# tl32rodan/DCVC

Hardware: AMD Instinct MI355X
Metric: encode+decode fps @1920x1080 per GPU; bpp bit-exact + PSNR Δ<1e-4 dB vs ref (higher is better)
Workload: dtype f32 (convs on split-fp16 f16x3 MFMA, fp32 accumulation); 1 GPU; C3 DCVC-DC RGB 1920x1080 (pad 1920x1088) IP=32 write mode; gop=32, precision=split, q_index=0, stream_part=8, parallelism=sequence-sharded x1, 3 GOP lane(s) per GPU, lanes=3, step=one frame on each of 3 lane(s)

## Files before the change

dcvc_amd/csrc/hip/slffn.hip:

```cpp
#include "common.h"
#include "split.h"

#include <cstring>

namespace {

constexpr int kNW = 4, kNT = kNW * 64;

constexpr int HS = 64;
#ifndef SLFFN_PB384
#define SLFFN_PB384 2
#endif
#ifndef SLDC_PB384
#define SLDC_PB384 2
#endif
constexpr int kOob = 0x7fffffe0;

struct LP {
  const float *x;
  int npix, xcs, xco, xbytes;
  float *y;
  int ycs, yco, ybytes;
  const uint16_t *w1, *w2;
  int w1bytes, w2bytes;
// ... 372 lines not shown
  return (c == 192 || c == 384) && hidden > 0 && hidden % HS == 0;
}

extern "C" int64_t dcvc_internal_lffn_pack(const float *w1, const float *w2, int c, int hidden, void *out) {
  if (!dcvc_internal_lffn_supported(c, hidden)) return DCVC_HIP_EINVAL;
  const int64_t n1 = (int64_t)hidden * c * 2, n2 = (int64_t)c * hidden * 2;
  if (!out) return n1 + n2;
  uint16_t *o = reinterpret_cast<uint16_t *>(out);
  pack_frags(w1, hidden, c, o);
  pack_frags(w2, c, hidden, o + n1);
  return n1 + n2;
}

extern "C" int dcvc_internal_lffn(const dcvc_ffn_args *a, void *stream) {
  if (!dcvc_internal_lffn_supported(a->c, a->hidden)) return DCVC_HIP_EUNSUPPORTED;
  const int64_t npix = (int64_t)a->x.H * a->x.W;
  if (npix <= 0) return DCVC_HIP_OK;
  auto bytes = [&](int cs, int co) { return (npix * cs - co) * 4; };
  if (bytes(a->x.cstride, a->x.coff) > 0x7fff0000 || bytes(a->y.cstride, a->y.coff) > 0x7fff0000)
    return DCVC_HIP_EUNSUPPORTED;
  LP p{};
  p.ovf = dcvc_internal_split_flag();
  p.x = reinterpret_cast<const float *>(a->x.ptr);
  p.npix = (int)npix;
  p.xcs = a->x.cstride;
  p.xco = a->x.coff;
  p.xbytes = (int)bytes(a->x.cstride, a->x.coff);
  p.y = reinterpret_cast<float *>(a->y.ptr);
  p.ycs = a->y.cstride;
  p.yco = a->y.coff;
  p.ybytes = (int)bytes(a->y.cstride, a->y.coff);
  const int64_t n1 = (int64_t)a->hidden * a->c * 2;
  p.w1 = reinterpret_cast<const uint16_t *>(a->w);
  p.w2 = p.w1 + n1;
  p.w1bytes = (int)(n1 * 2);
  p.w2bytes = (int)(n1 * 2);
  p.b1 = a->b1;
  p.b2 = a->b2;
  p.scale = a->scale;
  p.hidden = a->hidden;
  p.slope = a->slope;
  hipStream_t st = reinterpret_cast<hipStream_t>(stream);
  return a->c == 384 ? run<384, SLFFN_PB384>(p, st) : run<192, 2>(p, st);
}

extern "C" int64_t dcvc_frag_pack_weights(const float *w, int rows, int k, void *out) {
  if (!w || rows <= 0 || k <= 0 || rows % 16 || k % 32) return DCVC_HIP_EINVAL;
  if (out && !host_split_range_ok(w, (int64_t)rows * k)) return DCVC_HIP_EINVAL;
  const int64_t n = (int64_t)rows * k * 2;
  if (out) pack_frags(w, rows, k, reinterpret_cast<uint16_t *>(out));
  return n;
}

extern "C" int dcvc_dw_conv2_split(const dcvc_dwc_args *a, void *stream) {
  if (!a || !a->t.ptr || !a->r.ptr || !a->y.ptr || !a->w9 || !a->bdw || !a->w2 || !a->b2) return DCVC_HIP_EINVAL;
  const int c = a->c;
  if (a->t.dtype != DCVC_F32 || a->r.dtype != DCVC_F32 || a->y.dtype != DCVC_F32 || a->t.C != c || a->r.C != c ||
      a->y.C != c || a->t.H != a->y.H || a->t.W != a->y.W || a->r.H != a->y.H || a->r.W != a->y.W)
    return DCVC_HIP_EINVAL;
  if (c != 192 && c != 384 && c != 128) return DCVC_HIP_EUNSUPPORTED;
  auto al = [](const dcvc_tensor &v) { return (uintptr_t)v.ptr % 16 == 0 && v.cstride % 4 == 0 && v.coff % 4 == 0; };
  if (!al(a->t) || !al(a->r) || !al(a->y) || a->t.cstride % 8 || a->t.coff % 8) return DCVC_HIP_EUNSUPPORTED;
  const int64_t npix = (int64_t)a->t.H * a->t.W;
  if (npix <= 0) return DCVC_HIP_OK;
  auto bytes = [&](const dcvc_tensor &v) { return (npix * v.cstride - v.coff) * 4; };
  if (bytes(a->t) > 0x7fff0000 || bytes(a->r) > 0x7fff0000 || bytes(a->y) > 0x7fff0000) return DCVC_HIP_EUNSUPPORTED;
  DP p{};
  p.ovf = dcvc_internal_split_flag();
  p.t = reinterpret_cast<const float *>(a->t.ptr);
  p.npix = (int)npix;
  p.H = a->t.H;
  p.W = a->t.W;
  p.tcs = a->t.cstride;
  p.tco = a->t.coff;
  p.tbytes = (int)bytes(a->t);
  p.r = reinterpret_cast<const float *>(a->r.ptr);
  p.rcs = a->r.cstride;
  p.rco = a->r.coff;
  p.rbytes = (int)bytes(a->r);
  p.y = reinterpret_cast<float *>(a->y.ptr);
  p.ycs = a->y.cstride;
  p.yco = a->y.coff;
  p.ybytes = (int)bytes(a->y);
  p.w9 = a->w9;
  p.bdw = a->bdw;
  p.w2 = reinterpret_cast<const uint16_t *>(a->w2);
  p.w2bytes = (int)((int64_t)c * c * 2 * 2);
  p.b2 = a->b2;
  hipStream_t st = reinterpret_cast<hipStream_t>(stream);
  return c == 384 ? run_dc<384, SLDC_PB384>(p, st) : c == 192 ? run_dc<192, 2>(p, st) : run_dc<128, 2>(p, st);
}
```

dcvc_amd/hip.py:

```python
import ctypes
import os
import threading

import numpy as np
import torch

from ._native import NativeError, hip_lib, check

F32, BF16 = 0, 1
F16X3 = 2
ACT_NONE, ACT_LRELU, ACT_CLAMP01, ACT_ROUND = 0, 1, 2, 3
IN_NONE, IN_LRELU, IN_GATE = 0, 1, 2

_TORCH = {F32: torch.float32, BF16: torch.bfloat16}
_CNAME = {F32: "f32", BF16: "bf16", F16X3: "f16x3"}
_CODE = {torch.float32: F32, torch.bfloat16: BF16}


class CTensor(ctypes.Structure):
    _fields_ = [("ptr", ctypes.c_void_p), ("dtype", ctypes.c_int), ("H", ctypes.c_int),
                ("W", ctypes.c_int), ("C", ctypes.c_int), ("cstride", ctypes.c_int),
                ("coff", ctypes.c_int)]


class CDcbArgs(ctypes.Structure):
    _fields_ = [("x", CTensor), ("y", CTensor), ("cin", ctypes.c_int), ("cout", ctypes.c_int),
                ("gated", ctypes.c_int),
                ("w_conv1", ctypes.c_void_p), ("ld_conv1", ctypes.c_int), ("b_conv1", ctypes.c_void_p),
                ("w_dw", ctypes.c_void_p), ("b_dw", ctypes.c_void_p),
                ("w_conv2", ctypes.c_void_p), ("ld_conv2", ctypes.c_int), ("b_conv2", ctypes.c_void_p),
                ("w_adaptor", ctypes.c_void_p), ("ld_adaptor", ctypes.c_int), ("b_adaptor", ctypes.c_void_p),
                ("w_ffn1", ctypes.c_void_p), ("ld_ffn1", ctypes.c_int), ("b_ffn1", ctypes.c_void_p),
                ("w_ffn2", ctypes.c_void_p), ("ld_ffn2", ctypes.c_int), ("b_ffn2", ctypes.c_void_p),
                ("scale", ctypes.c_void_p), ("slope_dc", ctypes.c_float), ("slope_ffn", ctypes.c_float)]


class CConvArgs(ctypes.Structure):
    _fields_ = [("x", CTensor), ("y", CTensor), ("w", ctypes.c_void_p), ("bias", ctypes.c_void_p),
                ("cin", ctypes.c_int), ("cout", ctypes.c_int), ("kh", ctypes.c_int), ("kw", ctypes.c_int),
                ("stride", ctypes.c_int), ("pad", ctypes.c_int), ("compute", ctypes.c_int),
                ("in_op", ctypes.c_int), ("in_slope", ctypes.c_float), ("act", ctypes.c_int),
                ("slope", ctypes.c_float), ("shuffle", ctypes.c_int), ("scale", ctypes.c_void_p),
                ("res", CTensor), ("res2", CTensor)]


class CFfnArgs(ctypes.Structure):
    _fields_ = [("x", CTensor), ("y", CTensor), ("c", ctypes.c_int), ("hidden", ctypes.c_int),
                ("w", ctypes.c_void_p), ("b1", ctypes.c_void_p), ("b2", ctypes.c_void_p),
                ("scale", ctypes.c_void_p), ("slope", ctypes.c_float)]


class CDcArgs(ctypes.Structure):
    _fields_ = [("x", CTensor), ("y", CTensor), ("cin", ctypes.c_int), ("cout", ctypes.c_int),
                ("adaptor", ctypes.c_int), ("w", ctypes.c_void_p), ("b1", ctypes.c_void_p), ("wdw", ctypes.c_void_p),
                ("bdw", ctypes.c_void_p), ("b2", ctypes.c_void_p), ("ba", ctypes.c_void_p), ("slope", ctypes.c_float)]


class CDwcArgs(ctypes.Structure):
    _fields_ = [("t", CTensor), ("r", CTensor), ("y", CTensor), ("c", ctypes.c_int), ("w9", ctypes.c_void_p),
                ("bdw", ctypes.c_void_p), ("w2", ctypes.c_void_p), ("b2", ctypes.c_void_p)]


_T = CTensor
_vp, _i, _f = ctypes.c_void_p, ctypes.c_int, ctypes.c_float
HIP_SYMBOLS = [
    ("dcvc_conv_pack_weights", ctypes.c_int64, [_vp, _i, _i, _i, _i, _i, _vp]),
    ("dcvc_conv2d", _i, [ctypes.POINTER(CConvArgs), _vp]),
    ("dcvc_set_option", _i, [ctypes.c_char_p, _i]),
    ("dcvc_get_option", _i, [ctypes.c_char_p, ctypes.POINTER(_i)]),
    ("dcvc_split_range_flag", _i, [_vp]),
    ("dcvc_last_kernel", ctypes.c_char_p, []),
    ("dcvc_depthconv_block", _i, [ctypes.POINTER(CDcbArgs), _vp]),
    ("dcvc_ffn_pack_weights", ctypes.c_int64, [_vp, _vp, _i, _i, _vp]),
    ("dcvc_conv_ffn", _i, [ctypes.POINTER(CFfnArgs), _vp]),
    ("dcvc_dc_pack_weights", ctypes.c_int64, [_vp, _vp, _vp, _i, _i, _vp]),
    ("dcvc_depth_conv_split", _i, [ctypes.POINTER(CDcArgs), _vp]),
    ("dcvc_frag_pack_weights", ctypes.c_int64, [_vp, _i, _i, _vp]),
    ("dcvc_dw_conv2_split", _i, [ctypes.POINTER(CDwcArgs), _vp]),
    ("dcvc_dwconv3x3", _i, [_T, _T, _vp, _vp, _vp]),
    ("dcvc_flow_warp", _i, [_T, _T, _T, _vp, _vp, _vp]),
    ("dcvc_offset_diversity", _i, [_T, _T, _T, _T, _vp, _vp, _vp, _vp, _f, _vp]),
    ("dcvc_offset_diversity_workspace", ctypes.c_int64, [_i, _i]),
    ("dcvc_offset_diversity_ws", _i, [_T, _T, _T, _T, _vp, _vp, _vp, _vp, _f, _vp, ctypes.c_int64, _vp]),
    ("dcvc_resize2x", _i, [_T, _T, _i, _f, _vp]),
    ("dcvc_pool2x2", _i, [_T, _T, _i, _vp]),
    ("dcvc_add", _i, [_T, _T, _T, _vp]),
    ("dcvc_copy", _i, [_T, _T, _vp]),
    ("dcvc_pad_replicate", _i, [_T, _T, _vp]),
    ("dcvc_frame_to_nhwc", _i, [_vp, _i, _i, _T, _vp]),
    ("dcvc_frame_to_nhwc_zero_pad", _i, [_vp, _i, _i, _T, _vp]),
    ("dcvc_yuv420_to_nhwc", _i, [_vp, _vp, _i, _i, _T, _vp]),
    ("dcvc_frame_sse_workspace", ctypes.c_int64, []),
    ("dcvc_frame_sse", _i, [_T, _vp, _vp, _i, _i, _i, _vp, _vp, _vp]),
    ("dcvc_recon_to_u8", _i, [_T, _i, _i, _i, _vp, _vp]),
    ("dcvc_yuv420_to_rgb_nhwc", _i, [_vp, _vp, _i, _i, _T, _vp, _vp]),
    ("dcvc_rgb_to_yuv420_planes", _i, [_vp, _i, _i, _vp, _vp, _vp]),
    ("dcvc_yuv420f_to_nhwc", _i, [_vp, _vp, _i, _i, _T, _vp]),
    ("dcvc_frame_sse_f32", _i, [_T, _vp, _vp, _i, _i, _i, _vp, _vp, _vp]),
    ("dcvc_recon_to_u8_cross", _i, [_T, _i, _i, _i, _vp, _vp]),
    ("dcvc_quadtree_encode_step", _i, [_T, _T, _T, _i, _T, _T, _vp, _vp, _f, _f, _vp]),
    ("dcvc_quadtree_indexes_step", _i, [_T, _T, _i, _vp, _f, _f, _vp]),
    ("dcvc_quadtree_decode_step", _i, [_T, _T, _i, _vp, _T, _T, _vp]),
    ("dcvc_nhwc_to_symbols", _i, [_T, _vp, _vp]),
    ("dcvc_symbols_to_nhwc", _i, [_vp, _T, _vp]),
    ("dcvc_quadtree_estimate_step", _i, [_T, _T, _T, _i, _T, _T, _vp, _i, _vp]),
    ("dcvc_factorized_bits", _i, [_T, _vp, _vp, _vp]),
    ("dcvc_sum_f32", _i, [_vp, ctypes.c_int64, _vp, _vp]),
    ("dcvc_dual_prior_encode_step", _i, [_T, _T, _T, _i, _T, _vp, _vp, _vp, _f, _f, _vp]),
    ("dcvc_dual_prior_indexes_step", _i, [_T, _T, _i, _vp, _f, _f, _vp]),
    ("dcvc_dual_prior_decode_step", _i, [_T, _T, _i, _vp, _T, _vp, _vp]),
    ("dcvc_dual_prior_estimate_step", _i, [_T, _T, _T, _i, _T, _vp, _vp, _i, _f, _vp]),
    ("dcvc_channel_div", _i, [_T, _vp, _T, _vp]),
    ("dcvc_fill", _i, [_T, _f, _vp]),
# ... 318 lines not shown
        w1 = w1.detach().float().cpu().reshape(w1.shape[0], -1).contiguous().numpy()
        w2 = w2.detach().float().cpu().reshape(w2.shape[0], -1).contiguous().numpy()
        self.hidden, self.c = w1.shape
        dev = _device(device)
        self.w = _pack(lib().dcvc_ffn_pack_weights, w1, w2, self.c, self.hidden, device=dev)
        self.b1 = b1.detach().float().contiguous().to(dev)
        self.b2 = b2.detach().float().contiguous().to(dev)


class DcW:

    def __init__(self, w1, b1, w9c, bdw, w2, b2, wa=None, ba=None, device=None):
        f = lambda w: w.detach().float().cpu().reshape(w.shape[0], -1).contiguous().numpy()
        w1n, w2n = f(w1), f(w2)
        wan = f(wa) if wa is not None else None
        self.cin, self.cout = w1n.shape[0], w2n.shape[0]
        dev = _device(device)
        self.w = _pack(lib().dcvc_dc_pack_weights, w1n, w2n, wan, self.cin, self.cout, device=dev)
        g = lambda t: t.detach().float().contiguous().to(dev)
        self.b1, self.w9c, self.bdw, self.b2 = g(b1), g(w9c), g(bdw), g(b2)
        self.ba = g(ba) if wa is not None else None


class DwcW:

    def __init__(self, w9c, bdw, w2, b2, device=None):
        w = w2.detach().float().cpu().reshape(w2.shape[0], -1).contiguous().numpy()
        self.c = int(w.shape[0])
        dev = _device(device)
        self.w2 = _pack(lib().dcvc_frag_pack_weights, w, self.c, self.c, device=dev)
        g = lambda t: t.detach().float().contiguous().to(dev)
        self.w9c, self.bdw, self.b2 = g(w9c), g(bdw), g(b2)


def dw_conv2_split(dwc, t, r, y=None):
    if y is None:
        y = empty(t.H, t.W, dwc.c, F32, t.buf.device)
    a = CDwcArgs()
    a.t, a.r, a.y, a.c = t.c(), r.c(), y.c(), dwc.c
    a.w9, a.bdw, a.w2, a.b2 = dwc.w9c.data_ptr(), dwc.bdw.data_ptr(), dwc.w2.data_ptr(), dwc.b2.data_ptr()
    e0 = _t0()
    rc = lib().dcvc_dw_conv2_split(ctypes.byref(a), stream())
    if rc == UNSUPPORTED:
        return None
    check(rc, "dw_conv2_split")
    if e0 is not None:
        n = t.H * t.W
        kname = lib().dcvc_last_kernel().decode()
        _t1(e0, kname.split("<")[0], 2 * n * dwc.c * (9 + dwc.c), n * dwc.c * 4 * 3 + dwc.w2.numel() * 2,
            f"{kname} | dw+conv2 {dwc.c} {t.H}x{t.W} f16x3")
    return y


def depth_conv_split(dw, x, y=None, slope=0.01):
    if y is None:
        y = empty(x.H, x.W, dw.cout, F32, x.buf.device)
    a = CDcArgs()
    a.x, a.y = x.c(), y.c()
    a.cin, a.cout, a.adaptor = dw.cin, dw.cout, 1 if dw.ba is not None else 0
    a.w, a.b1, a.wdw, a.bdw, a.b2 = dw.w.data_ptr(), dw.b1.data_ptr(), dw.w9c.data_ptr(), dw.bdw.data_ptr(), \
        dw.b2.data_ptr()
    a.ba = dw.ba.data_ptr() if dw.ba is not None else None
    a.slope = slope
    e0 = _t0()
    r = lib().dcvc_depth_conv_split(ctypes.byref(a), stream())
    if r == UNSUPPORTED:
        return None
    check(r, "depth_conv_split")
    if e0 is not None:
        n = x.H * x.W
        kname = lib().dcvc_last_kernel().decode()
        fl = 2 * n * (dw.cin * dw.cin + 9 * dw.cin + dw.cin * dw.cout * (2 if dw.ba is not None else 1))
        _t1(e0, kname.split("<")[0], fl, n * (dw.cin + dw.cout) * 4 + dw.w.numel() * 2,
            f"{kname} | depthconv {dw.cin}->{dw.cout} {x.H}x{x.W} f16x3")
    return y


def conv_ffn(fw, x, y=None, scale=None, slope=0.1):
    if y is None:
        y = empty(x.H, x.W, x.C, F32, x.buf.device)
    a = CFfnArgs()
    a.x, a.y = x.c(), y.c()
    a.c, a.hidden = fw.c, fw.hidden
    a.w, a.b1, a.b2 = fw.w.data_ptr(), fw.b1.data_ptr(), fw.b2.data_ptr()
    a.scale = scale.data_ptr() if scale is not None else None
    a.slope = slope
    e0 = _t0()
    r = lib().dcvc_conv_ffn(ctypes.byref(a), stream())
    if r == UNSUPPORTED:
        return None
    check(r, "conv_ffn")
    if e0 is not None:
        n = x.H * x.W
        kname = lib().dcvc_last_kernel().decode()
        _t1(e0, kname.split("<")[0], 4 * n * fw.c * fw.hidden, n * fw.c * 4 * 3 + fw.w.numel() * 2,
            f"{kname} | ffn {fw.c}->{fw.hidden}->{fw.c} {x.H}x{x.W} f16x3")
    return y


def depthconv_block(blk, x, y, scale=None):
    a = CDcbArgs()
    a.x, a.y = x.c(), y.c()
    a.cin, a.cout, a.gated = blk.conv1.cin, blk.ffn2.cout, 1 if blk.gated else 0
    cp = lambda cw: (cw.w.data_ptr(), cw.w.numel() // cw.cout, cw.b.data_ptr())
    a.w_conv1, a.ld_conv1, a.b_conv1 = cp(blk.conv1)
    a.w_dw, a.b_dw = blk.dw[0].data_ptr(), blk.dw[1].data_ptr()
# ... 340 lines not shown
```

dcvc_amd/layers.py:

```python
import torch

from . import hip as K
from .hip import Act, F32, BF16, F16X3, ACT_LRELU, ACT_NONE, IN_LRELU, IN_GATE


FUSE_DCB = True
FUSE_FFN = True
FUSE_DC = True
DW128 = True
SDC_SHAPES = {(64, 48, True), (48, 32, True), (32, 64, True), (64, 64, False), (48, 48, False), (32, 32, False)}


class Precision:
    def __init__(self, feat, feat_compute, latent_compute):
        self.feat = feat
        self.feat_compute = feat_compute
        self.latent = F32
        self.latent_compute = latent_compute

    @staticmethod
    def parity():
        return Precision(F32, F32, F32)

    @staticmethod
    def fast(latent_compute=F32):
        return Precision(BF16, BF16, latent_compute)

    @staticmethod
    def split():
        return Precision(F32, F16X3, F16X3)

    @property
    def name(self):
        if self.feat_compute == F16X3:
            return "split"
        if self.feat == F32:
            return "parity"
        return "fast" if self.latent_compute == F32 else "fast-bf16-tail"


def split_checkpoint(codec, stage):
    if codec.prec.feat_compute == F16X3 and getattr(codec, "_guard_on", False):
        K.split_guard_check(f"{type(codec).__name__}.{stage}")


def parity_twin(codec):
    t = getattr(codec, "_parity_twin", None)
    if t is None:
        kw = dict(codec._init_kw, precision=Precision.parity(), device=codec.dev)
        t = type(codec)(**kw).load_state_dict(codec.sd)
        if codec.entropy_coder is not None:
            t.update(force=True)
        codec._parity_twin = t
    if codec.entropy_coder is not None:
        t.entropy_coder = codec.entropy_coder
    return t


def split_guarded(fn):
    import functools

    @functools.wraps(fn)
    def run(self, *args, **kw):
# ... 129 lines not shown
    def dw(self, name):
        w = self.take(name + ".weight").detach().float().cpu()
        C = w.shape[0]
        w9c = w.reshape(C, 9).t().contiguous().to(self.dev)
        b = self.take(name + ".bias").detach().float().contiguous().to(self.dev)
        return w9c, b

    def dtype(self, latent):
        return self.prec.latent if latent else self.prec.feat

    def fit(self, x, compute):
        if compute != BF16 and x.dtype != F32:
            return cast(x, F32)
        return x


def cast(x, dtype):
    if x.dtype == dtype:
        return x
    y = K.empty(x.H, x.W, x.C, dtype, x.buf.device)
    return K.copy(x, y)


class DepthConvBlock:

    def __init__(self, ctx, p, gated=False, latent=False, slope_dc=0.01, slope_ffn=0.1):
        self.ctx, self.latent, self.gated = ctx, latent, gated
        self.slope_dc, self.slope_ffn = slope_dc, slope_ffn
        d = p + ".block.0"
        f = p + ".block.1"
        self.conv1 = ctx.conv(d + ".conv1.0", latent=latent)
        self.dw = ctx.dw(d + ".depth_conv")
        self.conv2 = ctx.conv(d + ".conv2", latent=latent)
        self.adaptor = ctx.conv(d + ".adaptor", latent=latent) if ctx.has(d + ".adaptor") else None
        if gated:
            self.ffn1 = ctx.conv(f + ".conv", latent=latent)
            self.ffn2 = ctx.conv(f + ".conv_out", latent=latent)
        else:
            self.ffn1 = ctx.conv(f + ".conv.0", latent=latent)
            self.ffn2 = ctx.conv(f + ".conv.2", latent=latent)
        self.cout = self.ffn2.cout
        self.dcw = None
        sd = ctx.sd
        if (FUSE_DC and self.conv1.compute == F16X3 and not latent and
                (self.conv1.cin, self.conv2.cout, self.adaptor is not None) in SDC_SHAPES):
            self.dcw = K.DcW(sd[d + ".conv1.0.weight"], sd[d + ".conv1.0.bias"], self.dw[0], self.dw[1],
                             sd[d + ".conv2.weight"], sd[d + ".conv2.bias"],
                             sd[d + ".adaptor.weight"] if self.adaptor is not None else None,
                             sd[d + ".adaptor.bias"] if self.adaptor is not None else None, ctx.dev)
        self.dwc = None
        if (FUSE_DC and self.conv1.compute == F16X3 and self.adaptor is None and self.conv1.cin == self.conv2.cout
                and ((latent and self.conv2.cin in (192, 384)) or (DW128 and not latent and self.conv2.cin == 128))):
            self.dwc = K.DwcW(self.dw[0], self.dw[1], sd[d + ".conv2.weight"], sd[d + ".conv2.bias"], ctx.dev)
        self.ffn = None
        if (FUSE_FFN and not gated and self.ffn2.compute == F16X3 and self.cout in (32, 48, 64, 128, 192, 384)
                and self.ffn1.cout % (64 if self.cout != 128 else 32) == 0):
            sd = ctx.sd
            self.ffn = K.FfnW(sd[f + ".conv.0.weight"], sd[f + ".conv.0.bias"], sd[f + ".conv.2.weight"],
                              sd[f + ".conv.2.bias"], ctx.dev)

    def __call__(self, x, y=None, scale=None):
        ctx = self.ctx
        dt = ctx.dtype(self.latent)
        if (FUSE_DCB and not self.latent and x.dtype == BF16 and dt == BF16
                and self.conv1.compute == BF16 and self.cout <= 128 and x.C <= 128):
            out = y if y is not None else K.empty(x.H, x.W, self.cout, BF16, x.buf.device)
            if K.depthconv_block(self, x, out, scale) is not None:
                return out
        x = ctx.fit(x, self.conv1.compute)
        dc = None
        if self.dcw is not None:
            dc = K.depth_conv_split(self.dcw, x, slope=self.slope_dc)
        if dc is not None:
            pass
        elif self.adaptor is not None:
            idn = K.conv(self.adaptor, x, out_dtype=dt)
        else:
            idn = cast(x, dt)
        if dc is None:
            t = K.conv(self.conv1, x, out_dtype=dt, act=ACT_LRELU, slope=self.slope_dc)
            if self.dwc is not None:
                dc = K.dw_conv2_split(self.dwc, t, idn)
            if dc is None:
                t = K.dwconv3x3(t, *self.dw)
                dc = K.conv(self.conv2, t, res=idn)
        if self.gated:
            h = K.conv(self.ffn1, dc)
            return K.conv(self.ffn2, h, y, in_op=IN_GATE, in_slope=self.slope_ffn, res=dc, scale=scale)
        if self.ffn is not None:
            out = K.conv_ffn(self.ffn, dc, y, scale=scale, slope=self.slope_ffn)
            if out is not None:
                return out
        hid = BF16 if self.ffn2.compute == BF16 else dt
        h = K.conv(self.ffn1, dc, out_dtype=hid, act=ACT_LRELU, slope=self.slope_ffn)
        return K.conv(self.ffn2, h, y, out_dtype=dc.dtype, act=ACT_LRELU, slope=self.slope_ffn, res=dc,
                      scale=scale)


class ResidualBlockWithStride:

    def __init__(self, ctx, p, latent=False):
        self.ctx, self.latent = ctx, latent
        self.conv1 = ctx.conv(p + ".conv1", 2, latent)
        self.conv2 = ctx.conv(p + ".conv2", 1, latent)
        self.down = ctx.conv(p + ".downsample", 2, latent)

    def __call__(self, x, y=None, scale=None):
        dt = self.ctx.dtype(self.latent)
        x = self.ctx.fit(x, self.conv1.compute)
        t = K.conv(self.conv1, x, out_dtype=dt, act=ACT_LRELU, slope=0.01)
        idn = K.conv(self.down, x, out_dtype=dt)
        return K.conv(self.conv2, t, y, act=ACT_LRELU, slope=0.1, res=idn, scale=scale)


class ResidualBlockUpsample:

    def __init__(self, ctx, p, latent=False):
        self.ctx, self.latent = ctx, latent
        self.sub = ctx.conv(p + ".subpel_conv.0", 1, latent)
        self.conv = ctx.conv(p + ".conv", 1, latent)
        self.up = ctx.conv(p + ".upsample.0", 1, latent)

    def __call__(self, x, y=None, scale=None):
        dt = self.ctx.dtype(self.latent)
        x = self.ctx.fit(x, self.sub.compute)
        t = K.conv(self.sub, x, out_dtype=dt, shuffle=True, act=ACT_LRELU, slope=0.01)
        idn = K.conv(self.up, x, out_dtype=dt, shuffle=True)
        return K.conv(self.conv, t, y, act=ACT_LRELU, slope=0.1, res=idn, scale=scale)


class ResBlock:

    def __init__(self, ctx, p, slope=0.01, end_with_relu=False, latent=False):
# ... 116 lines not shown
```

include/dcvc_hip.h:

```cpp
#ifndef DCVC_HIP_H
#define DCVC_HIP_H

#include <stdint.h>

#ifdef __cplusplus
extern "C" {
#endif

#define DCVC_HIP_OK 0
#define DCVC_HIP_EINVAL (-1)
#define DCVC_HIP_ELAUNCH (-2)
#define DCVC_HIP_EUNSUPPORTED (-3)

enum dcvc_dtype { DCVC_F32 = 0, DCVC_BF16 = 1 };
#define DCVC_F16X3 2

enum dcvc_act {
  DCVC_ACT_NONE = 0,
  DCVC_ACT_LRELU = 1,
  DCVC_ACT_CLAMP01 = 2,
  DCVC_ACT_ROUND = 3
};

enum dcvc_in_op {
// ... 17 lines not shown
  const float *bias;
  int cin, cout;
  int kh, kw, stride, pad;
  int compute;
  int in_op;
  float in_slope;
  int act;
  float slope;
  int shuffle;
  const float *scale;
  dcvc_tensor res;
  dcvc_tensor res2;
} dcvc_conv_args;

int64_t dcvc_conv_pack_weights(const float *w, int cout, int cin, int kh,
                               int kw, int compute, void *out);
int dcvc_conv2d(const dcvc_conv_args *a, void *stream);
int dcvc_set_option(const char *name, int value);
int dcvc_get_option(const char *name, int *value);
int dcvc_split_range_flag(int *flag);
const char *dcvc_last_kernel(void);

typedef struct dcvc_dcb_args {
  dcvc_tensor x, y;
  int cin, cout, gated;
  const void *w_conv1; int ld_conv1; const float *b_conv1;
  const float *w_dw; const float *b_dw;
  const void *w_conv2; int ld_conv2; const float *b_conv2;
  const void *w_adaptor; int ld_adaptor; const float *b_adaptor;
  const void *w_ffn1; int ld_ffn1; const float *b_ffn1;
  const void *w_ffn2; int ld_ffn2; const float *b_ffn2;
  const float *scale;
  float slope_dc, slope_ffn;
} dcvc_dcb_args;
int dcvc_depthconv_block(const dcvc_dcb_args *a, void *stream);

typedef struct dcvc_ffn_args {
  dcvc_tensor x, y;
  int c, hidden;
  const void *w;
  const float *b1, *b2;
  const float *scale;
  float slope;
} dcvc_ffn_args;
int64_t dcvc_ffn_pack_weights(const float *w1, const float *w2, int c, int hidden, void *out);
int dcvc_conv_ffn(const dcvc_ffn_args *a, void *stream);

typedef struct dcvc_dwc_args {
  dcvc_tensor t, r, y;
  int c;
  const float *w9, *bdw;
  const void *w2;
  const float *b2;
} dcvc_dwc_args;
int64_t dcvc_frag_pack_weights(const float *w, int rows, int k, void *out);
int dcvc_dw_conv2_split(const dcvc_dwc_args *a, void *stream);

typedef struct dcvc_dc_args {
  dcvc_tensor x, y;
  int cin, cout, adaptor;
  const void *w;
  const float *b1, *wdw, *bdw, *b2, *ba;
  float slope;
} dcvc_dc_args;
int64_t dcvc_dc_pack_weights(const float *w1, const float *w2, const float *wa, int cin, int cout, void *out);
int dcvc_depth_conv_split(const dcvc_dc_args *a, void *stream);

int dcvc_dwconv3x3(dcvc_tensor x, dcvc_tensor y, const float *w,
                   const float *bias, void *stream);

int dcvc_flow_warp(dcvc_tensor x, dcvc_tensor flow, dcvc_tensor y,
                   const float *gx, const float *gy, void *stream);

int dcvc_offset_diversity(dcvc_tensor feat, dcvc_tensor offs_half,
                          dcvc_tensor flow, dcvc_tensor y, const float *fw,
                          const float *fb, const float *gx, const float *gy,
                          float max_mag, void *stream);

int64_t dcvc_offset_diversity_workspace(int H, int W);
int dcvc_offset_diversity_ws(dcvc_tensor feat, dcvc_tensor offs_half,
                             dcvc_tensor flow, dcvc_tensor y, const float *fw,
                             const float *fb, const float *gx, const float *gy,
                             float max_mag, void *workspace, int64_t ws_bytes,
                             void *stream);

int dcvc_resize2x(dcvc_tensor x, dcvc_tensor y, int up, float mul,
                  void *stream);
int dcvc_pool2x2(dcvc_tensor x, dcvc_tensor y, int is_max, void *stream);

int dcvc_add(dcvc_tensor a, dcvc_tensor b, dcvc_tensor y, void *stream);
int dcvc_copy(dcvc_tensor x, dcvc_tensor y, void *stream);
int dcvc_pad_replicate(dcvc_tensor x, dcvc_tensor y, void *stream);
int dcvc_frame_to_nhwc(const uint8_t *src, int h, int w, dcvc_tensor y,
                       void *stream);
int dcvc_frame_to_nhwc_zero_pad(const uint8_t *src, int h, int w, dcvc_tensor y,
                                void *stream);
int dcvc_yuv420_to_nhwc(const uint8_t *y, const uint8_t *uv, int h, int w,
                        dcvc_tensor out, void *stream);
int64_t dcvc_frame_sse_workspace(void);
int dcvc_frame_sse(dcvc_tensor x_hat, const uint8_t *src, const uint8_t *uv,
                   int h, int w, int yuv420, double *workspace, double *out3,
                   void *stream);
int dcvc_recon_to_u8(dcvc_tensor x_hat, int h, int w, int yuv420, uint8_t *out,
                     void *stream);

int dcvc_yuv420_to_rgb_nhwc(const uint8_t *y, const uint8_t *uv, int h, int w,
// ... 89 lines not shown
```

Before: 30.08 frames/s.

## Fuse depthwise 3x3, conv2, adaptor and residual into one split-fp16 tail kernel

Adds a persistent MFMA kernel that computes the depthwise 3x3 conv, the 1x1 conv2, an optional 1x1 adaptor on the block input, and the residual add in a single pass. It targets 128/64-channel non-latent depth-conv blocks. This removes the separate adaptor conv launch, the identity tensor round trip through memory, and the separate dw+conv2 path. LDS is double buffered and the next tile's halo loads are issued while the current stage computes. It adds new code paths only for three shape combinations.

After: 30.65 frames/s, median of 6. 1.02x the previous value.

```diff
diff --git a/dcvc_amd/csrc/hip/sdct.hip b/dcvc_amd/csrc/hip/sdct.hip
--- /dev/null
+++ b/dcvc_amd/csrc/hip/sdct.hip
@@ -0,0 +1,331 @@
+#include "common.h"
+#include "launch.h"
+#include "options.h"
+#include "split.h"
+
+namespace {
+
+constexpr int kNW = 8, kNT = kNW * 64;
+constexpr int TH = 8, TW = 16;
+constexpr int HWD = TW + 2;
+constexpr int HP = (TH + 2) * HWD;
+constexpr int TP = TH * TW;
+constexpr int kOob = 0x7fffffe0;
+
+struct TailP {
+  const float *t;
+  int H, W, tcs, tco, tbytes;
+  const float *x;
+  int xcs, xco, xbytes;
+  float *y;
+  int ycs, yco, ybytes;
+  const float *w9, *bdw, *b2, *ba;
+  const uint16_t *w2, *wa;
+  int txt, ntile;
+  int *ovf;
+};
+
+__device__ __forceinline__ __amdgpu_buffer_rsrc_t rsrc(const void *base, int bytes) {
+  return __builtin_amdgcn_make_buffer_rsrc(const_cast<void *>(base), (short)0, bytes, 0x00020000);
+}
+
+typedef uint32_t u32x2_t __attribute__((ext_vector_type(2)));
+
+template <int C, int CX, int COUT, bool ADAPT>
+constexpr size_t tail_lds() {
+  return (size_t)2 * HP * 32 * 4 + (size_t)4 * TP * 32 * 2 + (size_t)(10 * C + 2 * COUT) * 4;
+}
+
+template <int C, int CX, int COUT, bool ADAPT>
+__global__ void __launch_bounds__(kNT) sdct_kernel(TailP p) {
+  SplitRange rg(p.ovf);
+  constexpr int KA = ADAPT ? CX / 32 : 0, KC = C / 32, NS = KA + KC;
+  static_assert(NS % 2 == 0 && NS >= 2, "a tile starts in LDS buffer 0");
+  static_assert(ADAPT || (CX == C && COUT == C), "without an adaptor x is the identity");
+  constexpr int NRB = COUT / 16;
+  static_assert(kNW % NRB == 0, "a wave owns one row block");
+  constexpr int NPB = TH / (kNW / NRB);
+  extern __shared__ __align__(16) unsigned char smem[];
+  float *Hb = reinterpret_cast<float *>(smem);
+  uint16_t *Db = reinterpret_cast<uint16_t *>(Hb + 2 * HP * 32);
+  float *Lw9 = reinterpret_cast<float *>(Db + 4 * TP * 32);
+  float *Lbd = Lw9 + 9 * C;
+  float *Lb2 = Lbd + C, *Lba = Lb2 + COUT;
+
+  const int tid = threadIdx.x, lane = tid & 63;
+  const int wave = __builtin_amdgcn_readfirstlane(tid >> 6);
+  const int col = lane & 15, g = lane >> 4;
+  const int rb = wave % NRB, pb0 = (wave / NRB) * NPB;
+  const int G = gridDim.x;
+  const __amdgpu_buffer_rsrc_t tr = rsrc(p.t + p.tco, p.tbytes);
+  const __amdgpu_buffer_rsrc_t xr = rsrc(p.x + p.xco, p.xbytes);
+  const __amdgpu_buffer_rsrc_t yr = rsrc(p.y + p.yco, p.ybytes);
+
+  f16x8 w2h[KC], w2l[KC], wah[KA ? KA : 1], wal[KA ? KA : 1];
+  {
+    const __amdgpu_buffer_rsrc_t wr = rsrc(p.w2, COUT * C * 4);
+#pragma unroll
+    for (int kc = 0; kc < KC; ++kc) {
+      const int o = ((rb * KC + kc) * 1024 + lane * 8) * 2;
+      w2h[kc] = __builtin_bit_cast(f16x8, __builtin_amdgcn_raw_buffer_load_b128(wr, o, 0, 0));
+      w2l[kc] = __builtin_bit_cast(f16x8, __builtin_amdgcn_raw_buffer_load_b128(wr, o + 1024, 0, 0));
+    }
+    if constexpr (ADAPT) {
+      const __amdgpu_buffer_rsrc_t ar = rsrc(p.wa, COUT * CX * 4);
+#pragma unroll
+      for (int kc = 0; kc < KA; ++kc) {
+        const int o = ((rb * KA + kc) * 1024 + lane * 8) * 2;
+        wah[kc] = __builtin_bit_cast(f16x8, __builtin_amdgcn_raw_buffer_load_b128(ar, o, 0, 0));
+        wal[kc] = __builtin_bit_cast(f16x8, __builtin_amdgcn_raw_buffer_load_b128(ar, o + 1024, 0, 0));
+      }
+    }
+  }
+  const int n = rb * 16 + 4 * g;
+  for (int i = tid; i < 9 * C; i += kNT) Lw9[i] = p.w9[i];
+  for (int i = tid; i < C; i += kNT) Lbd[i] = p.bdw[i];
+  for (int i = tid; i < COUT; i += kNT) {
+    Lb2[i] = p.b2[i];
+    Lba[i] = ADAPT ? p.ba[i] : 0.f;
+  }
+
+  f32x4 pre[3];
+  auto issue = [&](int s, int y0, int x0) __attribute__((always_inline)) {
+    if (s < KA) {
+#pragma unroll
+      for (int i = 0; i < 2; ++i) {
+        const int u = tid + i * kNT, px = u >> 3, q = u & 7;
+        const int yy = y0 + (px >> 4), xx = x0 + (px & 15);
+        const bool ok = yy < p.H && xx < p.W;
+        const int o = ok ? ((yy * p.W + xx) * p.xcs + s * 32 + q * 4) * 4 : kOob;
+        pre[i] = __builtin_bit_cast(f32x4, __builtin_amdgcn_raw_buffer_load_b128(xr, o, 0, 0));
+      }
+    } else {
+#pragma unroll
+      for (int i = 0; i < 3; ++i) {
+        const int u = tid + i * kNT, hp = u >> 3, q = u & 7;
+        const int hy = hp / HWD, hx = hp - hy * HWD;
+        const int yy = y0 - 1 + hy, xx = x0 - 1 + hx;
+        const bool ok = u < HP * 8 && (unsigned)yy < (unsigned)p.H && (unsigned)xx < (unsigned)p.W;
+        const int o = ok ? ((yy * p.W + xx) * p.tcs + (s - KA) * 32 + q * 4) * 4 : kOob;
+        pre[i] = __builtin_bit_cast(f32x4, __builtin_amdgcn_raw_buffer_load_b128(tr, o, 0, 0));
+      }
+    }
+  };
+  auto stash = [&](int s) __attribute__((always_inline)) {
+    float *Hs = Hb + (s & 1) * HP * 32;
+#pragma unroll
+    for (int i = 0; i < (s < KA ? 2 : 3); ++i) {
+      const int u = tid + i * kNT;
+      if (i < 2 || u < HP * 8) *reinterpret_cast<f32x4 *>(Hs + u * 4) = pre[i];
+    }
+  };
+  auto put4 = [&](int s, int px, int q, const float *v) __attribute__((always_inline)) {
+    uint16_t *Dh = Db + (s & 1) * 2 * TP * 32, *Dl = Dh + TP * 32;
+    rg.add4(v);
+    const auto h0 = __builtin_amdgcn_cvt_pkrtz(v[0], v[1]);
+    const auto h1 = __builtin_amdgcn_cvt_pkrtz(v[2], v[3]);
+    const uint32_t l0 = pk(split_lo(v[0], (float)h0[0]), split_lo(v[1], (float)h0[1]));
+    const uint32_t l1 = pk(split_lo(v[2], (float)h1[0]), split_lo(v[3], (float)h1[1]));
+    const int off = swz(px, q >> 1) + (q & 1) * 4;
+    *reinterpret_cast<u32x2_t *>(Dh + off) = u32x2_t{__builtin_bit_cast(uint32_t, h0), __builtin_bit_cast(uint32_t, h1)};
+    *reinterpret_cast<u32x2_t *>(Dl + off) = u32x2_t{l0, l1};
+  };
+  auto image = [&](int s, int y0, int x0) __attribute__((always_inline)) {
+    const float *Hs = Hb + (s & 1) * HP * 32;
+    if (s < KA) {
+#pragma unroll
+      for (int i = 0; i < 2; ++i) {
+        const int u = tid + i * kNT;
+        const f32x4 a = *reinterpret_cast<const f32x4 *>(Hs + u * 4);
+        const float v[4] = {a[0], a[1], a[2], a[3]};
+        put4(s, u >> 3, u & 7, v);
+      }
+    } else {
+      const int q = tid & 7, cx = (tid >> 3) & 15, rp = tid >> 7;
+      const int c0 = (s - KA) * 32 + q * 4;
+      f32x4 wv[2][3];
+      float a0[4] = {0.f, 0.f, 0.f, 0.f}, a1[4] = {0.f, 0.f, 0.f, 0.f};
+#pragma unroll
+      for (int hr = 0; hr < 4; ++hr) {
+        if (hr < 3) {
+#pragma unroll
+          for (int dx = 0; dx < 3; ++dx)
+            wv[hr & 1][dx] = *reinterpret_cast<const f32x4 *>(Lw9 + (hr * 3 + dx) * C + c0);
+        }
+#pragma unroll
+        for (int dx = 0; dx < 3; ++dx) {
+          const f32x4 a = *reinterpret_cast<const f32x4 *>(Hs + ((2 * rp + hr) * HWD + cx + dx) * 32 + q * 4);
+          if (hr < 3) {
+#pragma unroll
+            for (int e = 0; e < 4; ++e) a0[e] = __builtin_fmaf(wv[hr & 1][dx][e], a[e], a0[e]);
+          }
+          if (hr > 0) {
+#pragma unroll
+            for (int e = 0; e < 4; ++e) a1[e] = __builtin_fmaf(wv[(hr - 1) & 1][dx][e], a[e], a1[e]);
+          }
+        }
+        sched_fence();
+      }
+      const f32x4 bd = *reinterpret_cast<const f32x4 *>(Lbd + c0);
+      const bool okx = x0 + cx < p.W;
+      const bool ok0 = okx && y0 + 2 * rp < p.H, ok1 = okx && y0 + 2 * rp + 1 < p.H;
+      float v0[4], v1[4];
+#pragma unroll
+      for (int e = 0; e < 4; ++e) {
+        v0[e] = ok0 ? a0[e] + bd[e] : 0.f;
+        v1[e] = ok1 ? a1[e] + bd[e] : 0.f;
+      }
+      put4(s, (2 * rp) * TW + cx, q, v0);
+      put4(s, (2 * rp + 1) * TW + cx, q, v1);
+    }
+  };
+
+  f32x4 am[NPB], ac[NPB], idn[NPB];
+#pragma unroll
+  for (int i = 0; i < NPB; ++i) {
+    am[i] = f32x4{0.f, 0.f, 0.f, 0.f};
+    ac[i] = f32x4{0.f, 0.f, 0.f, 0.f};
+    idn[i] = f32x4{0.f, 0.f, 0.f, 0.f};
+  }
+
+  int tile = blockIdx.x;
+  int ty = tile / p.txt;
+  int y0 = ty * TH, x0 = (tile - ty * p.txt) * TW;
+  issue(0, y0, x0);
+  stash(0);
+  issue(1, y0, x0);
+  __syncthreads();
+
+  for (; tile < p.ntile; tile += G) {
+    const int nxt = tile + G;
+    const bool more = nxt < p.ntile;
+    const int nty = nxt / p.txt;
+    const int ny0 = nty * TH, nx0 = (nxt - nty * p.txt) * TW;
+#pragma unroll
+    for (int s = 0; s < NS; ++s) {
+      image(s, y0, x0);
+      if (s + 1 < NS || more) stash((s + 1) % NS);
+      wait_lgkm();
+      raw_barrier();
+      if (s + 2 < NS)
+        issue(s + 2, y0, x0);
+      else if (more)
+        issue(s + 2 - NS, ny0, nx0);
+      if (!ADAPT && s == NS - 1) {
+#pragma unroll
+        for (int i = 0; i < NPB; ++i) {
+          const int yy = y0 + pb0 + i, xx = x0 + col;
+          const bool ok = yy < p.H && xx < p.W;
+          idn[i] = __builtin_bit_cast(
+              f32x4, __builtin_amdgcn_raw_buffer_load_b128(xr, ok ? ((yy * p.W + xx) * p.xcs + n) * 4 : kOob, 0, 0));
+        }
+      }
+      {
+        const uint16_t *Dh = Db + (s & 1) * 2 * TP * 32, *Dl = Dh + TP * 32;
+        const f16x8 ah = s < KA ? wah[s < KA ? s : 0] : w2h[s < KA ? 0 : s - KA];
+        const f16x8 al = s < KA ? wal[s < KA ? s : 0] : w2l[s < KA ? 0 : s - KA];
+#pragma unroll
+        for (int i = 0; i < NPB; ++i) {
+          const int o = swz((pb0 + i) * 16 + col, g);
+          const f16x8 bh = *reinterpret_cast<const f16x8 *>(Dh + o);
+          const f16x8 bl = *reinterpret_cast<const f16x8 *>(Dl + o);
+          am[i] = __builtin_amdgcn_mfma_f32_16x16x32_f16(ah, bh, am[i], 0, 0, 0);
+          ac[i] = __builtin_amdgcn_mfma_f32_16x16x32_f16(ah, bl, ac[i], 0, 0, 0);
+          ac[i] = __builtin_amdgcn_mfma_f32_16x16x32_f16(al, bh, ac[i], 0, 0, 0);
+          if ((i & 3) == 3) sched_fence();
+        }
+      }
+      if (ADAPT && s == KA - 1) {
+        const f32x4 bav = *reinterpret_cast<const f32x4 *>(Lba + n);
+#pragma unroll
+        for (int i = 0; i < NPB; ++i) {
+#pragma unroll
+          for (int e = 0; e < 4; ++e) idn[i][e] = (am[i][e] + ac[i][e] * kLoInv) + bav[e];
+          am[i] = f32x4{0.f, 0.f, 0.f, 0.f};
+          ac[i] = f32x4{0.f, 0.f, 0.f, 0.f};
+        }
+      }
+      if (s == NS - 1) {
+        const f32x4 b2v = *reinterpret_cast<const f32x4 *>(Lb2 + n);
+#pragma unroll
+        for (int i = 0; i < NPB; ++i) {
+          const int yy = y0 + pb0 + i, xx = x0 + col;
+          const bool ok = yy < p.H && xx < p.W;
+          f32x4 v;
+#pragma unroll
+          for (int e = 0; e < 4; ++e) v[e] = idn[i][e] + ((am[i][e] + ac[i][e] * kLoInv) + b2v[e]);
+          __builtin_amdgcn_raw_buffer_store_b128(__builtin_bit_cast(u32x4_t, v), yr,
+                                                 ok ? ((yy * p.W + xx) * p.ycs + n) * 4 : kOob, 0, 0);
+          am[i] = f32x4{0.f, 0.f, 0.f, 0.f};
+          ac[i] = f32x4{0.f, 0.f, 0.f, 0.f};
+        }
+      }
+    }
+    y0 = ny0;
+    x0 = nx0;
+  }
+}
+
+DCVC_OPTION("dctail", g_enable, 1);
+
+template <int C, int CX, int COUT, bool ADAPT>
+int run_tail(TailP p, hipStream_t st) {
+  constexpr size_t lds = tail_lds<C, CX, COUT, ADAPT>();
+  static_assert(lds <= 160 * 1024, "LDS of a CU");
+  const int cus = dcvc_cu_count();
+  if (cus <= 0) return DCVC_HIP_ELAUNCH;
+  const int G = p.ntile < cus ? p.ntile : cus;
+  auto kern = sdct_kernel<C, CX, COUT, ADAPT>;
+  dcvc_note_kernel("sdct_kernel<%d, %d, %d, %s>@%lld", C, CX, COUT, bname(ADAPT), (long long)G * kNT);
+  dcvc_ensure_lds(reinterpret_cast<const void *>(kern), 160 * 1024);
+  hipLaunchKernelGGL(kern, dim3((unsigned)G), dim3(kNT), lds, st, p);
+  DCVC_LAUNCH_CHECK();
+  return DCVC_HIP_OK;
+}
+
+}
+
+extern "C" int dcvc_internal_dctail(const dcvc_dwc_args *a, void *stream) {
+  if (!g_enable) return DCVC_HIP_EUNSUPPORTED;
+  const int c = a->c, cx = a->cx, cout = a->cout;
+  const bool adapt = a->wa != nullptr;
+  const bool inst = (c == 128 && cx == 128 && cout == 64 && adapt) || (c == 64 && cx == 64 && cout == 128 && adapt) ||
+                    (c == 128 && cx == 128 && cout == 128 && !adapt);
+  if (!inst) return DCVC_HIP_EUNSUPPORTED;
+  if (!f32_pieces_ok(a->t, 4) || !f32_pieces_ok(a->r, 4) || !f32_pieces_ok(a->y, 4)) return DCVC_HIP_EUNSUPPORTED;
+  auto al16 = [](const void *q) { return (uintptr_t)q % 16 == 0; };
+  if (!al16(a->w9) || !al16(a->bdw) || !al16(a->b2) || !al16(a->w2) || (adapt && (!al16(a->wa) || !al16(a->ba))))
+    return DCVC_HIP_EUNSUPPORTED;
+  const int64_t npix = (int64_t)a->t.H * a->t.W;
+  if (npix <= 0) return DCVC_HIP_OK;
+  auto bytes = [&](const dcvc_tensor &v) { return (npix * v.cstride - v.coff) * 4; };
+  if (bytes(a->t) > 0x7fff0000 || bytes(a->r) > 0x7fff0000 || bytes(a->y) > 0x7fff0000) return DCVC_HIP_EUNSUPPORTED;
+  TailP p{};
+  p.ovf = dcvc_internal_split_flag();
+  p.t = reinterpret_cast<const float *>(a->t.ptr);
+  p.H = a->t.H;
+  p.W = a->t.W;
+  p.tcs = a->t.cstride;
+  p.tco = a->t.coff;
+  p.tbytes = (int)bytes(a->t);
+  p.x = reinterpret_cast<const float *>(a->r.ptr);
+  p.xcs = a->r.cstride;
+  p.xco = a->r.coff;
+  p.xbytes = (int)bytes(a->r);
+  p.y = reinterpret_cast<float *>(a->y.ptr);
+  p.ycs = a->y.cstride;
+  p.yco = a->y.coff;
+  p.ybytes = (int)bytes(a->y);
+  p.w9 = a->w9;
+  p.bdw = a->bdw;
+  p.b2 = a->b2;
+  p.ba = a->ba;
+  p.w2 = reinterpret_cast<const uint16_t *>(a->w2);
+  p.wa = reinterpret_cast<const uint16_t *>(a->wa);
+  p.txt = (a->t.W + TW - 1) / TW;
+  p.ntile = p.txt * ((a->t.H + TH - 1) / TH);
+  hipStream_t st = reinterpret_cast<hipStream_t>(stream);
+  if (c == 128 && cout == 64) return run_tail<128, 128, 64, true>(p, st);
+  if (c == 64) return run_tail<64, 64, 128, true>(p, st);
+  return run_tail<128, 128, 128, false>(p, st);
+}
diff --git a/dcvc_amd/csrc/hip/slffn.hip b/dcvc_amd/csrc/hip/slffn.hip
--- a/dcvc_amd/csrc/hip/slffn.hip
+++ b/dcvc_amd/csrc/hip/slffn.hip
@@ -448,9 +448,20 @@
   return n;
 }
 
+extern "C" int dcvc_internal_dctail(const dcvc_dwc_args *a, void *stream);
+
 extern "C" int dcvc_dw_conv2_split(const dcvc_dwc_args *a, void *stream) {
   if (!a || !a->t.ptr || !a->r.ptr || !a->y.ptr || !a->w9 || !a->bdw || !a->w2 || !a->b2) return DCVC_HIP_EINVAL;
   const int c = a->c;
+  if (a->cx || a->cout) {
+    if (a->cx <= 0 || a->cout <= 0 || (a->wa != nullptr) != (a->ba != nullptr)) return DCVC_HIP_EINVAL;
+    if (!a->wa && (a->cx != c || a->cout != c)) return DCVC_HIP_EINVAL;
+    if (a->t.dtype != DCVC_F32 || a->r.dtype != DCVC_F32 || a->y.dtype != DCVC_F32 || a->t.C != c ||
+        a->r.C != a->cx || a->y.C != a->cout || a->t.H != a->y.H || a->t.W != a->y.W || a->r.H != a->y.H ||
+        a->r.W != a->y.W)
+      return DCVC_HIP_EINVAL;
+    return dcvc_internal_dctail(a, stream);
+  }
   if (a->t.dtype != DCVC_F32 || a->r.dtype != DCVC_F32 || a->y.dtype != DCVC_F32 || a->t.C != c || a->r.C != c ||
       a->y.C != c || a->t.H != a->y.H || a->t.W != a->y.W || a->r.H != a->y.H || a->r.W != a->y.W)
     return DCVC_HIP_EINVAL;
diff --git a/dcvc_amd/hip.py b/dcvc_amd/hip.py
--- a/dcvc_amd/hip.py
+++ b/dcvc_amd/hip.py
@@ -58,7 +58,8 @@
 
 class CDwcArgs(ctypes.Structure):
     _fields_ = [("t", CTensor), ("r", CTensor), ("y", CTensor), ("c", ctypes.c_int), ("w9", ctypes.c_void_p),
-                ("bdw", ctypes.c_void_p), ("w2", ctypes.c_void_p), ("b2", ctypes.c_void_p)]
+                ("bdw", ctypes.c_void_p), ("w2", ctypes.c_void_p), ("b2", ctypes.c_void_p),
+                ("cx", ctypes.c_int), ("cout", ctypes.c_int), ("wa", ctypes.c_void_p), ("ba", ctypes.c_void_p)]
 
 
 _T = CTensor
@@ -483,6 +484,47 @@
     return y
 
 
+class DcTailW:
+
+    def __init__(self, w9c, bdw, w2, b2, wa=None, ba=None, device=None):
+        f = lambda w: w.detach().float().cpu().reshape(w.shape[0], -1).contiguous().numpy()
+        w2n = f(w2)
+        self.cout, self.c = (int(s) for s in w2n.shape)
+        dev = _device(device)
+        self.w2 = _pack(lib().dcvc_frag_pack_weights, w2n, self.cout, self.c, device=dev)
+        g = lambda t: t.detach().float().contiguous().to(dev)
+        self.w9c, self.bdw, self.b2 = g(w9c), g(bdw), g(b2)
+        self.cx, self.wa, self.ba = self.c, None, None
+        if wa is not None:
+            wan = f(wa)
+            self.cx = int(wan.shape[1])
+            self.wa = _pack(lib().dcvc_frag_pack_weights, wan, self.cout, self.cx, device=dev)
+            self.ba = g(ba)
+
+
+def dc_tail_split(tw, t, x, y=None):
+    if y is None:
+        y = empty(t.H, t.W, tw.cout, F32, t.buf.device)
+    a = CDwcArgs()
+    a.t, a.r, a.y, a.c, a.cx, a.cout = t.c(), x.c(), y.c(), tw.c, tw.cx, tw.cout
+    a.w9, a.bdw, a.w2, a.b2 = tw.w9c.data_ptr(), tw.bdw.data_ptr(), tw.w2.data_ptr(), tw.b2.data_ptr()
+    if tw.wa is not None:
+        a.wa, a.ba = tw.wa.data_ptr(), tw.ba.data_ptr()
+    e0 = _t0()
+    rc = lib().dcvc_dw_conv2_split(ctypes.byref(a), stream())
+    if rc == UNSUPPORTED:
+        return None
+    check(rc, "dc_tail_split")
+    if e0 is not None:
+        n = t.H * t.W
+        kname = lib().dcvc_last_kernel().decode()
+        nw = tw.w2.numel() + (tw.wa.numel() if tw.wa is not None else 0)
+        fl = 2 * n * (9 * tw.c + tw.c * tw.cout + (tw.cx * tw.cout if tw.wa is not None else 0))
+        _t1(e0, kname.split("<")[0], fl, n * (tw.c + tw.cx + tw.cout) * 4 + nw * 2,
+            f"{kname} | dctail {tw.c}+{tw.cx}->{tw.cout} {t.H}x{t.W} f16x3")
+    return y
+
+
 def depth_conv_split(dw, x, y=None, slope=0.01):
     if y is None:
         y = empty(x.H, x.W, dw.cout, F32, x.buf.device)
diff --git a/dcvc_amd/layers.py b/dcvc_amd/layers.py
--- a/dcvc_amd/layers.py
+++ b/dcvc_amd/layers.py
@@ -9,6 +9,7 @@
 FUSE_DC = True
 DW128 = True
 SDC_SHAPES = {(64, 48, True), (48, 32, True), (32, 64, True), (64, 64, False), (48, 48, False), (32, 32, False)}
+SDCT_SHAPES = {(128, 64, True), (64, 128, True), (128, 128, False)}
 
 
 class Precision:
@@ -244,6 +245,12 @@
         if (FUSE_DC and self.conv1.compute == F16X3 and self.adaptor is None and self.conv1.cin == self.conv2.cout
                 and ((latent and self.conv2.cin in (192, 384)) or (DW128 and not latent and self.conv2.cin == 128))):
             self.dwc = K.DwcW(self.dw[0], self.dw[1], sd[d + ".conv2.weight"], sd[d + ".conv2.bias"], ctx.dev)
+        self.dct = None
+        if (FUSE_DC and self.conv1.compute == F16X3 and not latent and
+                (self.conv1.cin, self.conv2.cout, self.adaptor is not None) in SDCT_SHAPES):
+            self.dct = K.DcTailW(self.dw[0], self.dw[1], sd[d + ".conv2.weight"], sd[d + ".conv2.bias"],
+                                 sd[d + ".adaptor.weight"] if self.adaptor is not None else None,
+                                 sd[d + ".adaptor.bias"] if self.adaptor is not None else None, ctx.dev)
         self.ffn = None
         if (FUSE_FFN and not gated and self.ffn2.compute == F16X3 and self.cout in (32, 48, 64, 128, 192, 384)
                 and self.ffn1.cout % (64 if self.cout != 128 else 32) == 0):
@@ -263,14 +270,12 @@
         dc = None
         if self.dcw is not None:
             dc = K.depth_conv_split(self.dcw, x, slope=self.slope_dc)
-        if dc is not None:
-            pass
-        elif self.adaptor is not None:
-            idn = K.conv(self.adaptor, x, out_dtype=dt)
-        else:
-            idn = cast(x, dt)
         if dc is None:
             t = K.conv(self.conv1, x, out_dtype=dt, act=ACT_LRELU, slope=self.slope_dc)
+            if self.dct is not None and dt == F32 and x.dtype == F32:
+                dc = K.dc_tail_split(self.dct, t, x)
+        if dc is None:
+            idn = K.conv(self.adaptor, x, out_dtype=dt) if self.adaptor is not None else cast(x, dt)
             if self.dwc is not None:
                 dc = K.dw_conv2_split(self.dwc, t, idn)
             if dc is None:
diff --git a/include/dcvc_hip.h b/include/dcvc_hip.h
--- a/include/dcvc_hip.h
+++ b/include/dcvc_hip.h
@@ -93,6 +93,9 @@
   const float *w9, *bdw;
   const void *w2;
   const float *b2;
+  int cx, cout;
+  const void *wa;
+  const float *ba;
 } dcvc_dwc_args;
 int64_t dcvc_frag_pack_weights(const float *w, int rows, int k, void *out);
 int dcvc_dw_conv2_split(const dcvc_dwc_args *a, void *stream);
```
